# SamsungLabs/fcaf3d

Measured on AMD Instinct MI355X. Metric: scenes/sec fwd+bwd, ScanNet 100k-pt 2cm voxels, 1/2/4/8 MI355X, higher is better.
Workload: dtype f32

## Files before the change

### fcaf3d_amd/csrc/conv.hip

```cpp
#include "fc_common.h"
#include "../../include/fcaf3d_hip.h"
#ifdef FC_TRACE
__device__ unsigned long long* g_trace_buf_lds;
__device__ int g_trace_cap_lds;
extern "C" int fc_debug_trace_lds(unsigned long long* buf, int cap) {
  FC_HIP(hipMemcpyToSymbol(HIP_SYMBOL(g_trace_buf_lds), &buf, sizeof(buf)));
  FC_HIP(hipMemcpyToSymbol(HIP_SYMBOL(g_trace_cap_lds), &cap, sizeof(cap)));
  return FC_OK;
}
#define TR_BUF g_trace_buf_lds
#define TR_CAP g_trace_cap_lds
#endif
#include "fc_trace.h"

typedef float f32x16 __attribute__((ext_vector_type(16)));
typedef float f32x2 __attribute__((ext_vector_type(2)));
typedef float f32x4 __attribute__((ext_vector_type(4)));

__device__ __attribute__((aligned(16))) float g_zero_row[64];

__device__ int g_fc_prio;
extern "C" int fc_debug_set_prio(int mode) {
  FC_HIP(hipMemcpyToSymbol(HIP_SYMBOL(g_fc_prio), &mode, sizeof(mode)));
  return FC_OK;
}

static int g_bf16_fast = 0;
extern "C" int fc_set_bf16_fast(int on) {
  g_bf16_fast = on ? 1 : 0;
  return FC_OK;
}

static int g_split_mode = 2;
static inline int split_mode() { return g_bf16_fast ? 0 : g_split_mode; }
extern "C" int fc_set_split_mode(int mode) {
  if (mode != 0 && mode != 2) return FC_EINVAL;
  g_split_mode = mode;
  return FC_OK;
}
extern "C" int fc_get_split_mode(void) { return split_mode(); }
static int g_h3r = 1;
extern "C" int fc_debug_set_h3r(int mode) {
  if (mode < 0 || mode > 2) return FC_EINVAL;
  g_h3r = mode;
  return FC_OK;
}

#include <mutex>
#include "conv_tile.h"
#include "conv_f32.h"
#include "wgrad_f32.h"
#include "conv_stem.h"
#include "conv_x6.h"
#include "wgrad_x6.h"
#include "conv_h3r.h"
#include "conv_route.h"
static inline RouteEnv route_env() { return {split_mode(), g_bf16_fast, g_h3r}; }

__global__ __launch_bounds__(256) void k_amax(const f32x4* __restrict__ x, int64_t n4, const float* __restrict__ tail, int ntail,
                                              unsigned* __restrict__ slot) {
  __shared__ unsigned wm[4];
  __shared__ int last_s;
  unsigned m = 0u;
  const int64_t stride = (int64_t)gridDim.x * 256;
  for (int64_t i = (int64_t)blockIdx.x * 256 + threadIdx.x; i < n4; i += 4 * stride) {
    f32x4 v[4];
#pragma unroll
    for (int q = 0; q < 4; ++q) v[q] = i + q * stride < n4 ? x[i + q * stride] : f32x4{0.f, 0.f, 0.f, 0.f};
#pragma unroll
    for (int q = 0; q < 4; ++q)
#pragma unroll
      for (int j = 0; j < 4; ++j) { const unsigned u = __float_as_uint(v[q][j]) & 0x7fffffffu; m = (u > m && u < 0x7f800000u) ? u : m; }
  }
  if (blockIdx.x == 0 && (int)threadIdx.x < ntail) { const unsigned u = __float_as_uint(tail[threadIdx.x]) & 0x7fffffffu; m = (u > m && u < 0x7f800000u) ? u : m; }
#pragma unroll
  for (int off = 32; off > 0; off >>= 1) { const unsigned o = (unsigned)__shfl_xor((int)m, off, 64); m = o > m ? o : m; }
  if ((threadIdx.x & 63) == 0) wm[threadIdx.x >> 6] = m;
  __syncthreads();
  if (threadIdx.x == 0) {
    unsigned b = wm[0];
    for (int w = 1; w < 4; ++w) b = wm[w] > b ? wm[w] : b;
    if (b > __hip_atomic_load(&slot[1], __ATOMIC_RELAXED, __HIP_MEMORY_SCOPE_AGENT)) atomicMax(&slot[1], b);
    __threadfence();
    last_s = atomicAdd(&slot[2], 1u) == gridDim.x - 1;
    if (last_s) {
      __threadfence();
      slot[0] = atomicExch(&slot[1], 0u);
      slot[2] = 0u;
    }
  }
}

constexpr int AMAX_RING = 2048;
static unsigned* g_amax_ring[16] = {};
static unsigned g_amax_next[16] = {};
static std::mutex g_amax_ring_mu;
static int amax_ring_slot(unsigned** slot) {
  int dev = 0;
  FC_HIP(hipGetDevice(&dev));
  if (dev < 0 || dev >= 16) return FC_EINVAL;
  std::lock_guard<std::mutex> lock(g_amax_ring_mu);
  if (!g_amax_ring[dev]) {
    FC_HIP(hipMalloc((void**)&g_amax_ring[dev], (size_t)AMAX_RING * FC_AMAX_SLOT_BYTES));
    FC_HIP(hipMemset(g_amax_ring[dev], 0, (size_t)AMAX_RING * FC_AMAX_SLOT_BYTES));
  }
  const unsigned i = __atomic_fetch_add(&g_amax_next[dev], 1u, __ATOMIC_RELAXED) % AMAX_RING;
  *slot = g_amax_ring[dev] + (size_t)i * (FC_AMAX_SLOT_BYTES / 4);
  return FC_OK;
}
static int amax_launch(const float* x, int64_t n, unsigned* slot, hipStream_t stream) {
  if (n <= 0) { FC_HIP(hipMemsetAsync(slot, 0, 4, stream)); return FC_OK; }
  const int64_t n4 = n / 4;
  int64_t blocks = fc_cdiv(n4 > 0 ? n4 : 1, 256 * 8);
  if (blocks > 1024) blocks = 1024;
  k_amax<<<(unsigned)blocks, 256, 0, stream>>>(reinterpret_cast<const f32x4*>(x), n4, x + 4 * n4, (int)(n - 4 * n4), slot);
  FC_CHECK_LAUNCH();
  return FC_OK;
}
static thread_local const unsigned* t_amax_hint[2] = {nullptr, nullptr};
struct AmaxHintScope { ~AmaxHintScope() { t_amax_hint[0] = t_amax_hint[1] = nullptr; } };
static int operand_amax(const float* x, int64_t n, int which, hipStream_t stream, const unsigned** out) {
  const unsigned* h = t_amax_hint[which];
  if (h) { *out = h; return FC_OK; }
  unsigned* slot;
  int rc = amax_ring_slot(&slot);
  if (rc) return rc;
  rc = amax_launch(x, n, slot, stream);
  *out = slot;
  return rc;
}
extern "C" int fc_amax(const float* x, int64_t n, unsigned* slot, hipStream_t stream) {
  if (!slot || n < 0 || (n > 0 && !x) || ((uintptr_t)x & 15)) return FC_EINVAL;
  return amax_launch(x, n, slot, stream);
}
extern "C" int fc_conv_amax_hint(const unsigned* amax_in, const unsigned* amax_gout) {
  t_amax_hint[0] = amax_in;
  t_amax_hint[1] = amax_gout;
  return FC_OK;
}

// ... 83 lines not shown
__global__ __launch_bounds__(256) void k_sum_parts_stats(const float* __restrict__ part, float* __restrict__ out, int64_t n, int C, int S,
                                                         int RB, X6Epi epi) {
  __shared__ f32x4 sm[16 * 2 * 16];
  const int lane = threadIdx.x & 15, rl = threadIdx.x >> 4;
  const int64_t r0 = (int64_t)blockIdx.x * RB;
  const int c = blockIdx.y * 64 + lane * 4;
  const StatCh p = stat_channels(epi, c);
  f32x4 a1 = {0.f, 0.f, 0.f, 0.f}, a2 = a1;
  for (int64_t r = r0 + rl; r < r0 + RB && r < n; r += 16) {
    f32x4 a = *reinterpret_cast<const f32x4*>(part + r * C + c);
    for (int z = 1; z < S; ++z) a += *reinterpret_cast<const f32x4*>(part + ((int64_t)z * n + r) * C + c);
    *reinterpret_cast<f32x4*>(out + r * C + c) = a;
    stat_accumulate(p, epi, a, r * C + c, a1, a2);
  }
  stat_block_reduce(a1, a2, epi.stats, C, sm);
}

__global__ __launch_bounds__(256) void k_sum_pairs_stats(const float* __restrict__ part, const int* __restrict__ pos, float* __restrict__ out,
                                                         int64_t n_out, int K, int Cout, int RB, X6Epi epi) {
  __shared__ f32x4 sm[16 * 2 * 16];
  const int lane = threadIdx.x & 15, rl = threadIdx.x >> 4;
  const int64_t r0 = (int64_t)blockIdx.x * RB;
  const int c = blockIdx.y * 64 + lane * 4;
  const StatCh p = stat_channels(epi, c);
  f32x4 a1 = {0.f, 0.f, 0.f, 0.f}, a2 = a1;
  const int64_t rend = (r0 + RB < n_out) ? r0 + RB : n_out;
  for (int64_t o = r0 + rl; o < rend; o += 32) {
    const int64_t o2 = o + 16;
    const bool two = o2 < rend;
    f32x4 a = {0.f, 0.f, 0.f, 0.f}, b = a;
    for (int k0 = 0; k0 < K; k0 += 9) {
      int j[9], j2[9];
#pragma unroll
      for (int u = 0; u < 9; ++u) {
        j[u] = k0 + u < K ? pos[(int64_t)(k0 + u) * n_out + o] : -1;
        j2[u] = (two && k0 + u < K) ? pos[(int64_t)(k0 + u) * n_out + o2] : -1;
      }
      f32x4 v[9], v2[9];
#pragma unroll
      for (int u = 0; u < 9; ++u) {
        const float* src = j[u] >= 0 ? part + ((int64_t)(k0 + u) * n_out + j[u]) * Cout + c : g_zero_row + lane * 4;
        const float* src2 = j2[u] >= 0 ? part + ((int64_t)(k0 + u) * n_out + j2[u]) * Cout + c : g_zero_row + lane * 4;
        v[u] = *reinterpret_cast<const f32x4*>(src);
        v2[u] = *reinterpret_cast<const f32x4*>(src2);
      }
#pragma unroll
      for (int u = 0; u < 9; ++u) {
        if (j[u] >= 0) a += v[u];
        if (j2[u] >= 0) b += v2[u];
      }
    }
    *reinterpret_cast<f32x4*>(out + o * Cout + c) = a;
    stat_accumulate(p, epi, a, o * Cout + c, a1, a2);
    if (two) {
      *reinterpret_cast<f32x4*>(out + o2 * Cout + c) = b;
      stat_accumulate(p, epi, b, o2 * Cout + c, a1, a2);
    }
  }
  stat_block_reduce(a1, a2, epi.stats, Cout, sm);
}

static_assert(STEM_CIN == 3 && STEM_COUT == 64 && BK == 32, "conv_route.h spells these shapes out");

struct ConvArgs {
  const float *in, *W; const int *nbr, *out_index, *cnt; float* dst;
  int64_t n_rows; int K, Cin, Cout; X6Epi epi; hipStream_t stream;
};
#define FC_LAUNCH(...) __VA_ARGS__<<<grid, 256, 0, a.stream>>>(a.in, a.W, a.nbr, a.out_index, a.cnt, a.dst, a.n_rows, a.K, a.Cin, a.Cout)
#define FC_LAUNCH_EPI(...) __VA_ARGS__<<<grid, 256, 0, a.stream>>>(a.in, a.W, a.nbr, a.out_index, a.cnt, a.dst, a.n_rows, a.K, a.Cin, a.Cout, a.epi)

template <int BM, int BN, int WM>
static void launch_conv_fp32(const ConvRoute& r, const ConvArgs& a, dim3 grid) {
#define FC_LAUNCH_MFMA(KERNEL)                                                                                              \
  do { if (r.wsrc == FC_WSRC_FP32_T) FC_LAUNCH(KERNEL<BM, BN, 32, true, WM, true>); else if (a.nbr) FC_LAUNCH(KERNEL<BM, BN, 32, true, WM>); \
       else FC_LAUNCH(KERNEL<BM, BN, 32, false, WM>); } while (0)
  if (r.family == FC_FAM_MFMA) FC_LAUNCH_MFMA(k_conv_mfma);
  if constexpr (BM >= 128) {
    if (r.family == FC_FAM_MFMA_P) FC_LAUNCH_MFMA(k_conv_mfma_p);
    if (r.family == FC_FAM_GLDS) { if (a.nbr) FC_LAUNCH(k_conv_glds<BM, BN, true, WM>); else FC_LAUNCH(k_conv_glds<BM, BN, false, WM>); }
  }
#undef FC_LAUNCH_MFMA
}

template <int BM, int BN, int WM>
static void launch_conv_x6(const ConvRoute& r, const ConvArgs& a, dim3 grid) {
  if (r.family == FC_FAM_H3R) {
    if constexpr (BM == 128) {
      if (r.buf) FC_LAUNCH_EPI(k_conv_h3r<BN, true, true>);
      else if (a.nbr) FC_LAUNCH_EPI(k_conv_h3r<BN, true, false>);
      else FC_LAUNCH_EPI(k_conv_h3r<BN, false, false>);
    }
  } else if (r.wsrc == FC_WSRC_FP32_T) FC_LAUNCH_EPI(k_conv_x6<BM, BN, true, WM, 1>);
  else if (r.wsrc == FC_WSRC_FP32) { if (a.nbr) FC_LAUNCH_EPI(k_conv_x6<BM, BN, true, WM, 0>); else FC_LAUNCH_EPI(k_conv_x6<BM, BN, false, WM, 0>); }
  else if (r.mode == FC_MODE_BF16 || r.buf) {
    if constexpr (BM == 128) {
      if (r.mode == FC_MODE_BF16) { if (a.nbr) FC_LAUNCH_EPI(k_conv_x6<128, BN, true, 2, 2, 1>); else FC_LAUNCH_EPI(k_conv_x6<128, BN, false, 2, 2, 1>); }
      else if (r.mode == FC_MODE_H3) FC_LAUNCH_EPI(k_conv_x6<128, BN, true, 2, 2, 2, true>);
      else FC_LAUNCH_EPI(k_conv_x6<128, BN, true, 2, 2, 0, true>);
    }
  } else if (r.mode == FC_MODE_H3) { if (a.nbr) FC_LAUNCH_EPI(k_conv_x6<BM, BN, true, WM, 2, 2>); else FC_LAUNCH_EPI(k_conv_x6<BM, BN, false, WM, 2, 2>); }
  else { if (a.nbr) FC_LAUNCH_EPI(k_conv_x6<BM, BN, true, WM, 2>); else FC_LAUNCH_EPI(k_conv_x6<BM, BN, false, WM, 2>); }
}

static int launch_conv(const ConvRoute& r, const ConvArgs& a) {
  const dim3 grid(r.grid[0], r.grid[1], r.grid[2]);
  if (r.family == FC_FAM_STEM) {
    const size_t smem = (size_t)(STEM_ROWS * STEM_FWD_LDA + 96 * 64) * sizeof(float);
    k_stem_fwd<<<(unsigned)fc_cdiv(a.n_rows, STEM_ROWS), 256, smem, a.stream>>>(a.in, a.W, a.nbr, a.dst, nullptr, a.n_rows, a.K);
  } else if (r.family == FC_FAM_FMA) {
    k_conv_fma<<<(unsigned)fc_cdiv(a.n_rows * a.Cout, 256), 256, 0, a.stream>>>(a.in, a.W, a.nbr, a.dst, a.n_rows, a.K, a.Cin, a.Cout, r.wsrc == FC_WSRC_FP32_T ? 1 : 0);
  } else {
#define FC_TILE(BM, BN, WM) do { if (r.family >= FC_FAM_X6) launch_conv_x6<BM, BN, WM>(r, a, grid); else launch_conv_fp32<BM, BN, WM>(r, a, grid); } while (0)
    if (r.bm == 256) FC_TILE(256, 64, 4);
    else if (r.bm == 128 && r.bn == 128) FC_TILE(128, 128, 2);
    else if (r.bm == 128) FC_TILE(128, 64, 2);
    else if (r.bn == 128) launch_conv_fp32<64, 128, 2>(r, a, grid);
    else launch_conv_fp32<64, 64, 2>(r, a, grid);
#undef FC_TILE
  }
  FC_CHECK_LAUNCH();
  return FC_OK;
}
#undef FC_LAUNCH
#undef FC_LAUNCH_EPI

extern "C" {

int fc_conv_fwd_route(int64_t n_in, int64_t n_out, int K, int Cin, int Cout, int flags, int table_kind, int64_t live_tiles, int* out) {
  if (!out || n_in < 0 || n_out < 0 || K < 1 || Cin < 1 || Cout < 1) return FC_EINVAL;
  const ConvRoute r = conv_route({n_in, n_out, K, Cin, Cout}, flags, table_kind, live_tiles, route_env());
  const int f[16] = {r.family, r.bm, r.bn, r.wm, r.S, r.wsrc, r.mode, r.buf, r.epi, (int)r.grid[0], (int)r.grid[1], (int)r.grid[2]};
  for (int i = 0; i < 16; ++i) out[i] = f[i];
  return r.family == FC_FAM_INVALID ? FC_EINVAL : FC_OK;
}

int64_t fc_conv_fwd_ws_bytes(int64_t n_out, int K, int Cin, int Cout, int flags) {
  const ConvRoute r = conv_route({n_out, n_out, K, Cin, Cout}, flags, FC_TABLE_DENSE, 0, route_env());
  return r.S > 1 ? (int64_t)r.S * n_out * Cout * (int64_t)sizeof(float) : 0;
}

int64_t fc_conv_fwd_pairs_ws_bytes(int64_t n_out, int K, int Cout) {
  return (int64_t)K * n_out * Cout * (int64_t)sizeof(float);
}

int64_t fc_conv_stats_blocks(int64_t n_out, int K, int Cin, int Cout, int flags, int pairs) {
  if (n_out < 1) return 0;
  const ConvRoute r = conv_route({n_out, n_out, K, Cin, Cout}, flags, pairs ? FC_TABLE_PAIRS : FC_TABLE_DENSE, 0, route_env());
  if (r.epi == FC_EPI_NONE) return 0;
  return r.epi == FC_EPI_SUM ? fc_cdiv(n_out, fc_stat_rb(n_out)) : fc_cdiv(n_out, r.bm);
}

static int conv_impl(const float* in, const float* W, const int* nbr, const int* out_index, const int* cnt, const int* pos, float* out,
                     int64_t n_in, int64_t n_out, int K, int Cin, int Cout, int64_t live_tiles, int flags, void* ws, int64_t ws_bytes,
                     hipStream_t stream, const X6Epi* epi) {
  AmaxHintScope hint_scope;
  if (n_in < 0 || n_out < 0 || K < 1 || Cin < 1 || Cout < 1) return FC_EINVAL;
  if (n_out == 0 && !cnt) return epi ? FC_EINVAL : FC_OK;
  if (out_index && !nbr) return FC_EINVAL;
  const int table = cnt ? FC_TABLE_PAIRS : out_index ? FC_TABLE_SORTED : nbr ? FC_TABLE_DENSE : FC_TABLE_NONE;
  const ConvRoute r = conv_route({n_in, n_out, K, Cin, Cout}, flags, table | (epi ? FC_TABLE_STATS : 0), live_tiles, route_env());
  if (r.family == FC_FAM_INVALID) return FC_EINVAL;
  if (n_out == 0) return FC_OK;
  ConvArgs a = {in, W, nbr, out_index, cnt, out, n_out, K, Cin, Cout, {}, stream};
  if (r.family == FC_FAM_STEM || r.family == FC_FAM_FMA) return launch_conv(r, a);
  const bool parts = cnt || r.S > 1;
  if (parts && ws_bytes < (int64_t)r.S * n_out * Cout * (int64_t)sizeof(float)) return FC_EWS;
  if (parts) a.dst = (float*)ws;
  if (epi && r.epi == FC_EPI_KERNEL) a.epi = *epi;
  int rc = FC_OK;
  if (r.mode == FC_MODE_H3) rc = operand_amax(in, n_in * (int64_t)Cin, 0, stream, &a.epi.amax_in);
  if (rc == FC_OK) rc = launch_conv(r, a);
  if (rc != FC_OK || !parts) return rc;
  const int rb = fc_stat_rb(n_out);
  const dim3 sgrid((unsigned)fc_cdiv(n_out, rb), Cout / 64);
  if (cnt && epi) k_sum_pairs_stats<<<sgrid, 256, 0, stream>>>(a.dst, pos, out, n_out, K, Cout, rb, *epi);
  else if (cnt) k_sum_pairs<<<(unsigned)fc_cdiv(n_out * (Cout / 4), 256), 256, 0, stream>>>(a.dst, pos, out, n_out, K, Cout);
  else if (epi) k_sum_parts_stats<<<sgrid, 256, 0, stream>>>(a.dst, out, n_out, Cout, r.S, rb, *epi);
  else k_sum_parts<<<(unsigned)fc_cdiv(n_out * Cout / 4, 256), 256, 0, stream>>>(a.dst, out, n_out * Cout / 4, r.S);
  FC_CHECK_LAUNCH();
  return FC_OK;
}

static int conv_pairs_impl(const float* in, const float* W, const int* pair_in, const int* pair_cnt, const int* pair_pos, float* out,
                           int64_t n_in, int64_t n_out, int K, int Cin, int Cout, int64_t live_tiles, int flags, void* ws,
                           int64_t ws_bytes, hipStream_t stream, const X6Epi* epi) {
  if (!pair_in || !pair_cnt || !pair_pos || K > 65535) return FC_EINVAL;
  return conv_impl(in, W, pair_in, nullptr, pair_cnt, pair_pos, out, n_in, n_out, K, Cin, Cout, live_tiles, flags, ws, ws_bytes, stream, epi);
}

static X6Epi stats_epi(float* stats, const float* bn_x = nullptr, const float* mean = nullptr, const float* var = nullptr, const float* gamma = nullptr,
                       const float* beta = nullptr, float eps = 0.f, int act = 0, const float* add = nullptr, const float* bn_y = nullptr) {
  return {stats, bn_x, mean, var, gamma, beta, eps, act, add, bn_y, nullptr};
}

int fc_conv_fwd(const float* in, const float* W, const int* nbr, const int* out_index, float* out, int64_t n_in,
                int64_t n_out, int K, int Cin, int Cout, int flags, void* ws, int64_t ws_bytes, hipStream_t stream) {
// ... 311 lines not shown
```

### fcaf3d_amd/csrc/conv_h3r.h

```cpp
#pragma once

template <int BN, bool HAS_NBR, bool BUF>
__global__ __launch_bounds__(256, BN == 64 ? 4 : 3) void k_conv_h3r(
    const float* __restrict__ in, const float* __restrict__ W, const int* __restrict__ nbr,
    const int* __restrict__ out_index, const int* __restrict__ cnt, float* __restrict__ out, int64_t n_out, int K, int Cin,
    int Cout, X6Epi epi) {
  constexpr int BM = 128;
  constexpr int TN = BN / 32;
  constexpr int NG = BN / 64;
  constexpr int GU = 2 * 64 * 4;
  constexpr int BU = 3 * BN / 64;
  __shared__ u32x4 Bs[2][NG * GU];
  __shared__ unsigned int kmask_s;
  float* __restrict__ stats = epi.stats;

  const int tid = threadIdx.x, lane = tid & 63;
  const int wave = __builtin_amdgcn_readfirstlane(tid >> 6);
  const int r = lane & 31, h = lane >> 5;
  int64_t bx = blockIdx.x;
  const int n0 = blockIdx.y * BN;
  int S = gridDim.z, z = blockIdx.z;
  int kbase = 0;
  if (cnt) {
    const PairTile pt = tile_pair_walk<BM>(cnt, K, bx, z);
    bx = pt.bx; z = pt.z;
    const int64_t stride = n_out;
    n_out = cnt[z];
    if (bx * BM >= n_out) return;
    nbr += (int64_t)z * stride;
    kbase = z;
    out += (int64_t)z * stride * Cout;
    K = 1; S = 1; z = 0;
  }
  const int64_t m0 = bx * BM;
  const float h3_sa = h3_scale(fc_amax_read(epi.amax_in));
  const float h3_inv = h3_unscale(h3_sa, h3_scale(fc_amax_read(reinterpret_cast<const unsigned*>(W) + X6_IMG_AMAX_WORD)));

  f32x16 acc[TN];
#pragma unroll
  for (int j = 0; j < TN; ++j)
#pragma unroll
    for (int e = 0; e < 16; ++e) acc[j][e] = 0.f;

  const unsigned int kmask = (unsigned int)__builtin_amdgcn_readfirstlane((int)tile_offset_mask<BM, HAS_NBR>(&kmask_s, nbr, m0, n_out, z, K, S, tid, lane));
  constexpr unsigned X6_DEAD = 0x80000000u;

  if (kmask) {
    const int nst = __popc(kmask) * (Cin / 32);
    unsigned int rem = kmask;
    int lk = __ffs(rem) - 1;
    rem &= rem - 1;
    int lnk = rem ? __ffs(rem) - 1 : lk;
    if (rem) rem &= rem - 1;
    int lc0 = 0;
    bool sw = false;
    f32x4 av[4];
    u32x4 bi[BU];
    int vcur, vnxt;
    const int rows_here = (int)((n_out - m0) < BM ? (n_out - m0) : BM);
    const int lrow = wave * 32 + r;
    const __amdgpu_buffer_rsrc_t rn = __builtin_amdgcn_make_buffer_rsrc(const_cast<int*>(nbr), 0, 0x7fffffff, 0x00020000);
    const unsigned irow = (lrow < rows_here ? (unsigned)(m0 + lrow) : 0u) * 4u;
    auto fetch_idx = [&](int kk) -> int {
      if (BUF && HAS_NBR) return (int)__builtin_amdgcn_raw_buffer_load_b32(rn, (int)irow, (int)((unsigned)kk * (unsigned)n_out * 4u), 0);
      const int64_t row = lrow < rows_here ? m0 + lrow : 0;
      return HAS_NBR ? nbr[(int64_t)kk * n_out + row] : (int)row;
    };
    vcur = fetch_idx(lk);
    vnxt = fetch_idx(lnk);
    unsigned ocur = 0u;
    auto row_offset = [&]() {
      ocur = (vcur >= 0 && lrow < rows_here) ? (unsigned)vcur * (unsigned)(Cin * 4) + (unsigned)(h * 32) : X6_DEAD;
    };
    if (BUF) row_offset();
    const __amdgpu_buffer_rsrc_t ra = __builtin_amdgcn_make_buffer_rsrc(const_cast<float*>(in), 0, (int)X6_DEAD, 0x00020000);
    const __amdgpu_buffer_rsrc_t rb = __builtin_amdgcn_make_buffer_rsrc(const_cast<float*>(W), 0, -1, 0x00020000);
    const u32x4* img = reinterpret_cast<const u32x4*>(W);
    const int nslab = Cin / 32, ngrp = Cout / 64;
    auto load_stage = [&]() {
      if (sw) {
        sw = false;
        lk = lnk;
        vcur = vnxt;
        if (rem) {
          lnk = __ffs(rem) - 1;
          rem &= rem - 1;
        }
        vnxt = fetch_idx(lnk);
        if (BUF) row_offset();
      }
      if (BUF) {
        const unsigned boff = (((unsigned)(kbase + lk) * (unsigned)nslab + (unsigned)(lc0 / 32)) * (unsigned)ngrp + (unsigned)(n0 / 64)) * (unsigned)(X6_GROUP_U16 * 16);
#pragma unroll
        for (int i = 0; i < BU; ++i)
          if (i % 3 != 2) bi[i] = __builtin_amdgcn_raw_buffer_load_b128(rb, tid * 16, (int)(boff + 4096u * i), 0);
#pragma unroll
        for (int q = 0; q < 4; ++q)
          av[q] = __builtin_bit_cast(f32x4, __builtin_amdgcn_raw_buffer_load_b128(ra, (int)(ocur + (unsigned)(64 * (q >> 1) + 16 * (q & 1))), lc0 * 4, 0));
        return;
      }
      const u32x4* src = img + (((int64_t)(kbase + lk) * nslab + lc0 / 32) * ngrp + n0 / 64) * X6_GROUP_U16 + tid;
#pragma unroll
      for (int i = 0; i < BU; ++i)
        if (i % 3 != 2) bi[i] = src[256 * i];
      const bool live = vcur >= 0 && lrow < rows_here;
      const float* rowp = live ? in + (int64_t)vcur * Cin + lc0 + 8 * h : g_zero_row;
#pragma unroll
      for (int q = 0; q < 4; ++q) av[q] = *reinterpret_cast<const f32x4*>(rowp + (live ? 16 * (q >> 1) + 4 * (q & 1) : 4 * q));
    };
    u32x4 fa[2][2];
    auto split_rows = [&]() {
#pragma unroll
      for (int b = 0; b < 2; ++b) {
        unsigned p0[4], p1[4];
#pragma unroll
        for (int q = 0; q < 2; ++q) {
          h3_split2s(av[2 * b + q][0], av[2 * b + q][1], h3_sa, p0[2 * q], p1[2 * q]);
          h3_split2s(av[2 * b + q][2], av[2 * b + q][3], h3_sa, p0[2 * q + 1], p1[2 * q + 1]);
        }
        fa[b][0] = u32x4{p0[0], p0[1], p0[2], p0[3]};
        fa[b][1] = u32x4{p1[0], p1[1], p1[2], p1[3]};
      }
    };
    auto store_weights = [&](int buf) {
#pragma unroll
      for (int i = 0; i < BU; ++i)
        if (i % 3 != 2) Bs[buf][(i / 3) * GU + (i % 3) * 256 + tid] = bi[i];
    };
    load_stage();
    store_weights(0);
    split_rows();
    const int swz = (r >> 2) & 3;
    int b_slot[2];
#pragma unroll
    for (int b = 0; b < 2; ++b) b_slot[b] = r * 4 + ((2 * b + h) ^ swz);
    for (int st = 0; st < nst; ++st) {
      const int cur = st & 1;
      __syncthreads();
      if (st + 1 < nst) {
        lc0 += 32;
        if (lc0 >= Cin) {
          lc0 = 0;
          sw = true;
        }
      }
      load_stage();
      __builtin_amdgcn_sched_barrier(0);
#pragma unroll
      for (int b = 0; b < 2; ++b) {
#pragma unroll
        for (int pb = 1; pb >= 0; --pb) {
          u32x4 fb[TN];
#pragma unroll
          for (int j = 0; j < TN; ++j) fb[j] = Bs[cur][(j >> 1) * GU + pb * 256 + (j & 1) * 32 * 4 + b_slot[b]];
#pragma unroll
          for (int pa = 1 - pb; pa >= 0; --pa)
#pragma unroll
            for (int j = 0; j < TN; ++j) acc[j] = H3_MFMA(fa[b][pa], fb[j], acc[j]);
        }
      }
      store_weights(cur ^ 1);
      split_rows();
    }
  }
#pragma unroll
  for (int j = 0; j < TN; ++j)
#pragma unroll
    for (int e = 0; e < 16; ++e) acc[j][e] *= h3_inv;

  float* dst = out + (int64_t)z * n_out * Cout + n0 + 2 * r;
  int orow[16];
#pragma unroll
  for (int e = 0; e < 16; ++e) {
    const int64_t row = m0 + wave * 32 + (e & 3) + 8 * (e >> 2) + 4 * h;
    int o = -1;
    if (row < n_out) o = out_index ? out_index[row] : (int)row;
    orow[e] = o;
  }
  if (stats) {
    const bool bwd = epi.bn_x != nullptr;
    const bool from_y = bwd && epi.bn_y != nullptr && epi.act != 0;
    float mu[TN], is[TN], ga[TN], be[TN];
#pragma unroll
    for (int j = 0; j < TN; ++j) {
      const int col = n0 + (j >> 1) * 64 + 2 * r + (j & 1);
      mu[j] = 0.f; is[j] = 1.f; ga[j] = 1.f; be[j] = 0.f;
      if (bwd) {
        mu[j] = epi.mean[col];
        is[j] = 1.f / sqrtf(epi.var[col] + epi.eps);
        ga[j] = epi.gamma ? epi.gamma[col] : 1.f;
        be[j] = epi.beta ? epi.beta[col] : 0.f;
      }
    }
    float s1[TN], s2[TN];
#pragma unroll
    for (int j = 0; j < TN; ++j) { s1[j] = 0.f; s2[j] = 0.f; }
#pragma unroll
    for (int e0 = 0; e0 < 16; e0 += 4) {
      float xv[4][TN], av2[4][TN], yv[4][TN];
#pragma unroll
      for (int u = 0; u < 4; ++u) {
        const int o = orow[e0 + u];
#pragma unroll
        for (int j = 0; j < TN; ++j) { xv[u][j] = 0.f; av2[u][j] = 0.f; yv[u][j] = 0.f; }
        if (bwd && o >= 0) {
#pragma unroll
          for (int g = 0; g < NG; ++g) {
            const int64_t at = (int64_t)o * Cout + n0 + g * 64 + 2 * r;
            const f32x2 t = *reinterpret_cast<const f32x2*>(epi.bn_x + at);
            xv[u][2 * g] = t[0]; xv[u][2 * g + 1] = t[1];
            if (epi.add) { const f32x2 a2 = *reinterpret_cast<const f32x2*>(epi.add + at); av2[u][2 * g] = a2[0]; av2[u][2 * g + 1] = a2[1]; }
            if (from_y) { const f32x2 y2 = *reinterpret_cast<const f32x2*>(epi.bn_y + at); yv[u][2 * g] = y2[0]; yv[u][2 * g + 1] = y2[1]; }
          }
        }
      }
#pragma unroll
      for (int u = 0; u < 4; ++u) {
        if (bwd && orow[e0 + u] < 0) continue;
#pragma unroll
        for (int j = 0; j < TN; ++j) {
          float t1, t2;
          x6_epi_terms(bwd, bwd ? av2[u][j] + acc[j][e0 + u] : acc[j][e0 + u], xv[u][j], mu[j], is[j], ga[j], be[j], epi.act, from_y,
                       yv[u][j], t1, t2);
          s1[j] += t1;
          s2[j] += t2;
        }
      }
    }
#pragma unroll
    for (int j = 0; j < TN; ++j) {
      s1[j] += __shfl_xor(s1[j], 32, 64);
      s2[j] += __shfl_xor(s2[j], 32, 64);
    }
    __syncthreads();
    float* red = reinterpret_cast<float*>(&Bs[0][0]);
    if (h == 0) {
#pragma unroll
      for (int j = 0; j < TN; ++j) {
        const int cl = (j >> 1) * 64 + 2 * r + (j & 1);
        red[(wave * BN + cl) * 2 + 0] = s1[j];
        red[(wave * BN + cl) * 2 + 1] = s2[j];
      }
    }
    __syncthreads();
    if (tid < BN) {
      float a = 0.f, b = 0.f;
#pragma unroll
      for (int w = 0; w < 4; ++w) { a += red[(w * BN + tid) * 2 + 0]; b += red[(w * BN + tid) * 2 + 1]; }
      stats[((int64_t)blockIdx.x * 2 + 0) * Cout + n0 + tid] = a;
      stats[((int64_t)blockIdx.x * 2 + 1) * Cout + n0 + tid] = b;
    }
  }
#pragma unroll
  for (int e = 0; e < 16; ++e) {
    if (orow[e] >= 0) {
#pragma unroll
      for (int g = 0; g < NG; ++g) {
        f32x2 v = {acc[2 * g][e], acc[2 * g + 1][e]};
        *reinterpret_cast<f32x2*>(dst + (int64_t)orow[e] * Cout + g * 64) = v;
      }
    }
  }
}
```

### fcaf3d_amd/csrc/conv_route.h

```cpp
#ifndef FC_CONV_ROUTE_H
#define FC_CONV_ROUTE_H
#include "fc_common.h"
#include "../../include/fcaf3d_hip.h"

struct RouteEnv { int split_mode, bf16_fast, h3r; };
struct ConvShape { int64_t n_in, n_out; int K, Cin, Cout; };

struct ConvRoute {
  int family;
  int bm, bn, wm;
  int S;
  int wsrc, mode, buf, epi;
  unsigned grid[3];
};
struct WgradRoute {
  int family;
  int bm, bn, ko, bkr;
  int table, mode, S;
  int64_t rps;
  int wbuf;
  unsigned grid_y;
};

static inline int flag_bm(int flags) { return (flags >> FC_CONV_BM_SHIFT) & FC_CONV_TILE_MASK; }
static inline int flag_bn(int flags) { return (flags >> FC_CONV_BN_SHIFT) & FC_CONV_TILE_MASK; }
static inline int flag_s(int flags) { return (flags >> FC_CONV_S_SHIFT) & FC_CONV_S_MASK; }
static inline bool below_2gb(uint64_t bytes) { return bytes < (1ull << 31) - 4096u; }

static inline bool stem_shape(int K, int Cin, int Cout, int flags) { return !(flags & FC_CONV_FMA) && Cin == 3 && Cout == 64 && K <= 27; }

static inline int offset_split(int64_t tiles, int K) {
  if (K <= 1 || tiles >= 384) return 1;
  return (int)(1024 / tiles < K ? 1024 / tiles : K);
}

static inline ConvRoute conv_route(const ConvShape& s, int flags, int table, int64_t live_tiles, const RouteEnv& env) {
  const bool stats = (table & FC_TABLE_STATS) != 0;
  table &= ~FC_TABLE_STATS;
  const bool pairs = table == FC_TABLE_PAIRS, gather = table != FC_TABLE_NONE, split = (flags & FC_CONV_SPLIT) != 0;
  const bool image = split && (flags & FC_CONV_IMAGE);
  const bool wt = (flags & FC_CONV_WT) && !image;
  const int64_t n = s.n_out > 0 ? s.n_out : 1;
  const int K = s.K, Cin = s.Cin, Cout = s.Cout;
  ConvRoute r = {};
  r.family = FC_FAM_INVALID;
  r.wsrc = image ? FC_WSRC_IMAGE : wt ? FC_WSRC_FP32_T : FC_WSRC_FP32;
  if (!gather && (K != 1 || s.n_in != s.n_out)) return r;
  if ((flags & FC_CONV_WT) && !gather) return r;
  const bool mfma = Cin % 32 == 0 && Cout % 64 == 0 && (pairs || (!(flags & FC_CONV_FMA) && K <= 32));
  if (pairs && !mfma) return r;
  if (stats && !(mfma && split)) return r;
  r.bn = (Cout % 128 == 0) ? 128 : 64;
  if (pairs) {
    if (flag_bn(flags) == 1) r.bn = 64;
    r.bm = 128;
    r.S = K;
  } else {
    r.bm = (n > 64 && fc_cdiv(n, 128) * (Cout / r.bn) >= 4) ? 128 : 64;
    if (Cout == 64 && fc_cdiv(n, 256) >= 1024 && !split) r.bm = 256;
    const int fbm = flag_bm(flags), fbn = flag_bn(flags);
    if (fbm) r.bm = fbm == 1 ? 64 : (fbm == 2 ? 128 : 256);
    if (fbn && (Cout % (fbn == 1 ? 64 : 128) == 0)) r.bn = fbn == 1 ? 64 : 128;
    if (r.bm == 256) r.bn = 64;
    if (split && mfma && r.bm == 64) r.bm = 128;
    r.S = mfma ? offset_split(fc_cdiv(n, r.bm) * (Cout / r.bn), K) : 1;
    if (flag_s(flags)) r.S = flag_s(flags) > K ? K : flag_s(flags);
  }
  r.wm = r.bm == 256 ? 4 : 2;
  if (stem_shape(K, Cin, Cout, flags) && !(flags & FC_CONV_WT) && table == FC_TABLE_DENSE) { r.family = FC_FAM_STEM; return r; }
  if (!mfma && table != FC_TABLE_SORTED && !(flags & FC_CONV_IMAGE)) r.family = FC_FAM_FMA;
  if (!mfma) return r;
  r.grid[0] = (unsigned)fc_cdiv(n, r.bm), r.grid[1] = (unsigned)(Cout / r.bn), r.grid[2] = (unsigned)r.S;
  if (pairs && live_tiles > 0) r.grid[0] = (unsigned)live_tiles, r.grid[2] = 1;
  if (split) {
    r.family = FC_FAM_X6;
    r.mode = !image ? FC_MODE_SIX : (env.bf16_fast && r.bm == 128) ? FC_MODE_BF16 : env.split_mode == 2 ? FC_MODE_H3 : FC_MODE_SIX;
    if (r.mode == FC_MODE_H3 && r.bm == 128 && (env.h3r == 2 || (env.h3r == 1 && r.bn == 128))) r.family = FC_FAM_H3R;
    r.buf = image && gather && r.bm == 128 && r.mode != FC_MODE_BF16 && !(flags & FC_CONV_FLAT) &&
            below_2gb((uint64_t)s.n_in * (uint64_t)Cin * 4u) && below_2gb((uint64_t)K * (uint64_t)s.n_out * 4u);
    r.epi = (pairs || r.S > 1) ? FC_EPI_SUM : FC_EPI_KERNEL;
    return r;
  }
  const int64_t wgs = (int64_t)r.grid[0] * r.grid[1] * r.grid[2];
  r.mode = FC_MODE_FP32;
  if (flags & FC_CONV_GLDS) r.family = FC_FAM_GLDS;
  else if (flags & FC_CONV_PIPE_ON) r.family = FC_FAM_MFMA_P;
  else if ((flags & FC_CONV_PIPE_OFF) || (pairs && live_tiles <= 0)) r.family = FC_FAM_MFMA;
  else if (wgs >= 1536 || wgs <= 768) r.family = FC_FAM_MFMA_P;
  else r.family = (r.grid[2] > 1 && !(flags & FC_CONV_GLDS_OFF)) ? FC_FAM_GLDS : FC_FAM_MFMA;
  if (r.family == FC_FAM_GLDS && wt) r.family = FC_FAM_MFMA;
  if (r.bm == 64) r.family = FC_FAM_MFMA;
  return r;
}

#define WGRAD_KO 3

static inline WgradRoute wgrad_route(const ConvShape& s, int flags, int table, const RouteEnv& env) {
  const int64_t n = s.n_out > 0 ? s.n_out : 1;
  const int K = s.K, Cin = s.Cin, Cout = s.Cout, fbm = flag_bm(flags), fbn = flag_bn(flags);
  const bool dense = table == FC_TABLE_DENSE, pairs = table == FC_TABLE_PAIRS, split = (flags & FC_CONV_SPLIT) != 0;
  if (pairs) flags &= ~FC_CONV_WGRAD_DEEP;
  WgradRoute r = {};
  r.family = FC_WFAM_INVALID;
  r.table = table, r.ko = 1, r.bkr = 32, r.mode = FC_MODE_FP32;
  if (table == FC_TABLE_SORTED || (table == FC_TABLE_NONE && (K != 1 || s.n_in != s.n_out))) return r;
  const bool mfma = !(flags & FC_CONV_FMA) && Cin % 64 == 0 && Cout % 64 == 0;
  if (pairs && !mfma) return r;
  if (stem_shape(K, Cin, Cout, flags)) {
    r.family = dense ? FC_WFAM_STEM : FC_WFAM_FMA;
    r.rps = 1024, r.S = (int)fc_cdiv(n, 1024), r.grid_y = dense ? 1 : (unsigned)K;
    return r;
  }
  const bool multi = dense && mfma && !(flags & FC_CONV_WGRAD_MULTI_OFF) && K % WGRAD_KO == 0 && n >= 4096 &&
                     (!(flags & FC_CONV_WGRAD_MULTI_FIRST) || (Cin == 64 && n >= 32768));
  const bool x6t = mfma && split && (multi || !dense);
  const int wide = (Cout % 128 == 0) ? 128 : 64;
  r.bm = 64;
  r.bn = wide;
  if (fbm == 2 && Cin % 128 == 0) r.bm = 128;
  if (fbn == 1) r.bn = 64;
  if (fbn == 2 && Cout % 128 == 0) r.bn = 128;
  if (split && !dense && Cin % 128 == 0) r.bm = 128;
  int64_t sp = 1728 / (mfma ? (int64_t)K * (Cin / r.bm) * (Cout / r.bn) : (int64_t)K);
  if (multi) {
    constexpr int round_wide = 256, round_narrow = 512;
    sp = (wide == 128 ? round_wide : round_narrow) / ((int64_t)(K / WGRAD_KO) * (Cin / 64) * (Cout / wide));
  }
  const int64_t max_by_rows = fc_cdiv(n, mfma ? 512 : 2048);
  sp = sp > max_by_rows ? max_by_rows : sp;
  sp = sp > 256 ? 256 : sp < 1 ? 1 : sp;
  if (flag_s(flags)) sp = flag_s(flags);
  r.rps = fc_align(fc_cdiv(n, sp), 64);
  r.S = (int)fc_cdiv(n, r.rps);
  if (!mfma) { r.family = FC_WFAM_FMA, r.grid_y = (unsigned)K; return r; }
  if (x6t) {
    r.family = FC_WFAM_X6T;
    r.mode = env.bf16_fast ? FC_MODE_BF16 : env.split_mode == 2 ? FC_MODE_H3 : FC_MODE_SIX;
    r.bn = wide;
    if (multi) r.bm = 64, r.ko = WGRAD_KO;
    else if (r.bm == 128 && r.bn == 128 && (int64_t)r.S * K * (Cin / 128) * (Cout / 128) < 512) r.bm = 64;
    r.wbuf = !(flags & FC_CONV_FLAT) && below_2gb((uint64_t)s.n_in * (uint64_t)Cin * 4u) && below_2gb((uint64_t)s.n_out * (uint64_t)Cout * 4u) &&
             s.n_in < (1 << 24) && s.n_out < (1 << 24) && below_2gb((uint64_t)K * (uint64_t)s.n_out * 4u);
  } else if (multi) {
    r.family = FC_WFAM_MULTI, r.bm = 64, r.bn = wide, r.ko = WGRAD_KO;
  } else {
    if (pairs) r.bm = 64;
    const bool wpipe = r.bm == 64 && !(flags & FC_CONV_WGRAD_DEEP) && !(flags & FC_CONV_WGRAD_PIPE_OFF) &&
                       ((flags & FC_CONV_WGRAD_PIPE_ON) || (pairs && r.bn == 128));
    r.family = wpipe ? FC_WFAM_MFMA_P : FC_WFAM_MFMA;
    if (!wpipe && dense && (flags & FC_CONV_WGRAD_DEEP) && r.bm == 64) r.bkr = 64;
  }
  r.grid_y = (unsigned)((K / r.ko) * (Cin / r.bm) * (Cout / r.bn));
  return r;
}
#endif
```

### include/fcaf3d_hip.h

```cpp
#ifndef FCAF3D_HIP_H
#define FCAF3D_HIP_H
#include <stdint.h>

#ifndef __HIP_PLATFORM_AMD__
typedef struct ihipStream_t* hipStream_t;
#endif

#ifdef __cplusplus
extern "C" {
#endif

#define FC_ABI_VERSION 19
#ifndef FC_AMAX_SLOT_BYTES
#define FC_AMAX_SLOT_BYTES 2048
#endif
int fc_abi_version(void);


int fc_voxelize(const float* points, int64_t n, int pt_stride, int batch_idx, float voxel_size, float feat_div,
                int nfeat, int* coords, float* feats, hipStream_t stream);

int fc_augment_voxelize(const float* points, int64_t n_src, int pt_stride, const int* sample_idx, int64_t n_out,
                        const float* xform_host, int batch_idx, float voxel_size, float feat_div, int nfeat, int* coords,
                        float* feats, float* points_out, hipStream_t stream);
// ... 263 lines not shown
                      int kind, float* loss, float* iou, float* dpred, hipStream_t stream);

int fc_head_split_fwd(const float* y, int ld, const float* bias, const float* scale_dev, int64_t n, int n_reg, int n_cls,
                      float* centerness, float* bbox_pred, float* cls_score, float* cls_max, hipStream_t stream);
int fc_head_split_bwd(const float* y, int ld, const float* scale_dev, const float* bbox_pred, const float* g_centerness,
                      const float* g_bbox, const float* g_cls, int64_t n, int n_reg, int n_cls, float* gy,
                      float* gscale_row, hipStream_t stream);
int64_t fc_head_split_bwd_sums_ws_bytes(int64_t n);
int fc_head_split_bwd_sums(const float* y, int ld, const float* scale_dev, const float* bbox_pred, const float* g_centerness,
                           const float* g_bbox, const float* g_cls, int64_t n, int n_reg, int n_cls, float* gy, float* gbias,
                           float* gscale, void* ws, int64_t ws_bytes, hipStream_t stream);

int fc_sort_v(const float* vertices, const unsigned char* mask, const int* num_valid, int64_t n_pairs, int* idx,
              hipStream_t stream);

int64_t fc_assign_ws_bytes(int B, int M, int L);
int fc_assign_targets(const float* points, const int* scene, const int* level, int64_t N, const float* boxes,
                      const long long* labels, const int* box_count, int B, int M, int L, const int* order,
                      const int* seg_start, int limit, int topk, float* centerness_t, float* bbox_t, long long* labels_out,
                      void* ws, int64_t ws_bytes, hipStream_t stream);


int64_t fc_nms_bev_ws_bytes(int nseg, int stride);
int fc_nms_bev(const float* boxes, const int* counts_dev, int nseg, int stride, float thresh, int rotated,
               unsigned long long* mask_ws, int64_t ws_bytes, int* keep, int* keep_count, hipStream_t stream);
int fc_boxes_iou_bev(const float* boxes_a, int n, const float* boxes_b, int m, int rotated, float* out,
                     hipStream_t stream);


#define FC_MERGE_TO_BOTTOM 1
#define FC_MERGE_WITH_YAW 2
#define FC_MERGE_XF_FLIP_H (1ull << 32)
#define FC_MERGE_XF_FLIP_V (1ull << 33)
int64_t fc_merge_sorted_segments_ws_bytes(int nseg_out, int max_total);
int fc_merge_sorted_segments(const int64_t* desc, int nseg_out, int K, const int* counts_dev, const int* keep, int keep_stride,
                             const int64_t* ord, int ord_stride, const float* scores, int score_stride, const float* boxes,
                             int flags, int max_total, int cap, float* out_boxes, float* out_scores, int* out_src,
                             int* out_count, int stride_out, void* ws, int64_t ws_bytes, hipStream_t stream);


#define FC_VOTE_ROTATED 1
#define FC_VOTE_WITH_YAW 2
int fc_vote_boxes(const float* boxes, const float* scores, const int* counts_dev, int nseg, int stride, int max_count,
                  const int* keep, const int* keep_counts_dev, int keep_stride, int max_keep, float vote_thr, int flags,
                  float* out_boxes, int* out_members, hipStream_t stream);


#define FC_EVAL_DET_BOTTOM 1
int64_t fc_eval_match_ws_bytes(int64_t n_det, int64_t n_gt, int n_thr);
int fc_eval_match(const float* det_boxes, int det_dim , const float* det_scores, const int64_t* det_labels,
                  const float* gt_boxes , const int* gt_labels,
                  const int64_t* seg , int n_scenes,
                  int64_t n_det, int64_t n_gt, const double* thr , int n_thr, int flags,
                  float* best_iou, int* best_gt, unsigned char* tp_bits, void* ws, int64_t ws_bytes, hipStream_t stream);


int64_t fc_grad_norm_ws_bytes(int64_t n);
int fc_grad_norm(const float* g, int64_t n, float max_norm, float* out, void* ws, int64_t ws_bytes, hipStream_t stream);
int fc_adamw_step(float* p, const float* g, float* m, float* v, int64_t n, float lr, float beta1, float beta2, float eps,
                  float weight_decay, float bias_correction1, float bias_correction2, const float* norm_and_clip,
                  hipStream_t stream);

#define FC_ADAMW_MAX_RUNS 1024
int64_t fc_adamw_groups_table_bytes(int R);
int fc_adamw_groups_pack(const int64_t* begin, const float* lr_mult, const float* decay_mult, int R, int64_t n, void* out,
                         int64_t out_bytes);
int fc_adamw_step_groups(float* p, const float* g, float* m, float* v, int64_t n, float lr, float beta1, float beta2, float eps,
                         float weight_decay, float bias_correction1, float bias_correction2, const float* norm_and_clip,
                         const void* table_dev, int R, hipStream_t stream);

int fc_adamw_ema_step(float* p, const float* g, float* m, float* v, float* ema, int64_t n, float lr, float beta1, float beta2,
                      float eps, float weight_decay, float bias_correction1, float bias_correction2, const float* norm_and_clip,
                      const void* table_dev, int R, float ema_mu, float ema_keep, hipStream_t stream);
int fc_swap_f32(float* a, float* b, int64_t n, hipStream_t stream);

int fc_set_bf16_fast(int on);

int fc_set_split_mode(int mode);
int fc_get_split_mode(void);
int fc_amax(const float* x, int64_t n, unsigned* slot, hipStream_t stream);
int fc_conv_amax_hint(const unsigned* amax_in, const unsigned* amax_gout);
int fc_amax_out_hint(unsigned* amax_word);
int fc_debug_set_h3r(int mode);


int fc_exec_op_words(void);
int64_t fc_exec_probe_read(float* ms, int64_t* meta, int64_t cap);
int fc_exec_map_words(void);
int fc_exec(const int64_t* ops, int64_t op_begin, int64_t op_end, const int64_t* addr, const int64_t* dims, const int64_t* maps,
            const int64_t* streams, const int64_t* ws, const int64_t* ws_bytes, int64_t* ws_need, const int64_t* cfg);

#ifdef __cplusplus
}
#endif
#endif
```

Measured before the change: 538.5.

## Add 128x256 wide-N tile variant of h3r conv kernel for large wide shapes

Adds a BN=256 instantiation of the h3r split-precision conv kernel and routes wide, pair-driven convolutions with Cin>=256 and enough tiles to it, halving the grid along Cout. Wider N tiles reuse each gathered A fragment across twice as many MFMA columns, reducing gather/LDS traffic per FLOP. To limit register pressure the B-fragment loads and the BN-stats epilogue are processed in sub-groups, and occupancy is lowered to 2 waves per SIMD. It risks spills and lower occupancy hiding latency, and is controlled by a new debug knob.

```diff
diff --git a/fcaf3d_amd/csrc/conv.hip b/fcaf3d_amd/csrc/conv.hip
--- a/fcaf3d_amd/csrc/conv.hip
+++ b/fcaf3d_amd/csrc/conv.hip
@@ -43,6 +43,13 @@
 extern "C" int fc_debug_set_h3r(int mode) {
   if (mode < 0 || mode > 2) return FC_EINVAL;
   g_h3r = mode;
+  return FC_OK;
+}
+
+static int g_h3r_wide = 1;
+extern "C" int fc_debug_set_h3r_wide(int mode) {
+  if (mode < 0 || mode > 2) return FC_EINVAL;
+  g_h3r_wide = mode;
   return FC_OK;
 }
 
@@ -55,7 +62,7 @@
 #include "wgrad_x6.h"
 #include "conv_h3r.h"
 #include "conv_route.h"
-static inline RouteEnv route_env() { return {split_mode(), g_bf16_fast, g_h3r}; }
+static inline RouteEnv route_env() { return {split_mode(), g_bf16_fast, g_h3r, g_h3r_wide}; }
 
 __global__ __launch_bounds__(256) void k_amax(const f32x4* __restrict__ x, int64_t n4, const float* __restrict__ tail, int ntail,
                                               unsigned* __restrict__ slot) {
@@ -305,14 +312,17 @@
 #undef FC_LAUNCH_MFMA
 }
 
+template <int BN>
+static void launch_conv_h3r(const ConvRoute& r, const ConvArgs& a, dim3 grid) {
+  if (r.buf) FC_LAUNCH_EPI(k_conv_h3r<BN, true, true>);
+  else if (a.nbr) FC_LAUNCH_EPI(k_conv_h3r<BN, true, false>);
+  else FC_LAUNCH_EPI(k_conv_h3r<BN, false, false>);
+}
+
 template <int BM, int BN, int WM>
 static void launch_conv_x6(const ConvRoute& r, const ConvArgs& a, dim3 grid) {
   if (r.family == FC_FAM_H3R) {
-    if constexpr (BM == 128) {
-      if (r.buf) FC_LAUNCH_EPI(k_conv_h3r<BN, true, true>);
-      else if (a.nbr) FC_LAUNCH_EPI(k_conv_h3r<BN, true, false>);
-      else FC_LAUNCH_EPI(k_conv_h3r<BN, false, false>);
-    }
+    if constexpr (BM == 128) launch_conv_h3r<BN>(r, a, grid);
   } else if (r.wsrc == FC_WSRC_FP32_T) FC_LAUNCH_EPI(k_conv_x6<BM, BN, true, WM, 1>);
   else if (r.wsrc == FC_WSRC_FP32) { if (a.nbr) FC_LAUNCH_EPI(k_conv_x6<BM, BN, true, WM, 0>); else FC_LAUNCH_EPI(k_conv_x6<BM, BN, false, WM, 0>); }
   else if (r.mode == FC_MODE_BF16 || r.buf) {
@@ -335,6 +345,7 @@
   } else {
 #define FC_TILE(BM, BN, WM) do { if (r.family >= FC_FAM_X6) launch_conv_x6<BM, BN, WM>(r, a, grid); else launch_conv_fp32<BM, BN, WM>(r, a, grid); } while (0)
     if (r.bm == 256) FC_TILE(256, 64, 4);
+    else if (r.bn == 256) launch_conv_h3r<256>(r, a, grid);
     else if (r.bm == 128 && r.bn == 128) FC_TILE(128, 128, 2);
     else if (r.bm == 128) FC_TILE(128, 64, 2);
     else if (r.bn == 128) launch_conv_fp32<64, 128, 2>(r, a, grid);
diff --git a/fcaf3d_amd/csrc/conv_h3r.h b/fcaf3d_amd/csrc/conv_h3r.h
--- a/fcaf3d_amd/csrc/conv_h3r.h
+++ b/fcaf3d_amd/csrc/conv_h3r.h
@@ -1,13 +1,15 @@
 #pragma once
 
 template <int BN, bool HAS_NBR, bool BUF>
-__global__ __launch_bounds__(256, BN == 64 ? 4 : 3) void k_conv_h3r(
+__global__ __launch_bounds__(256, BN == 64 ? 4 : BN == 256 ? 2 : 3) void k_conv_h3r(
     const float* __restrict__ in, const float* __restrict__ W, const int* __restrict__ nbr,
     const int* __restrict__ out_index, const int* __restrict__ cnt, float* __restrict__ out, int64_t n_out, int K, int Cin,
     int Cout, X6Epi epi) {
   constexpr int BM = 128;
   constexpr int TN = BN / 32;
   constexpr int NG = BN / 64;
+  constexpr int FG = 4;
+  constexpr int SJ = 2;
   constexpr int GU = 2 * 64 * 4;
   constexpr int BU = 3 * BN / 64;
   __shared__ u32x4 Bs[2][NG * GU];
@@ -150,13 +152,26 @@
       for (int b = 0; b < 2; ++b) {
 #pragma unroll
         for (int pb = 1; pb >= 0; --pb) {
-          u32x4 fb[TN];
-#pragma unroll
-          for (int j = 0; j < TN; ++j) fb[j] = Bs[cur][(j >> 1) * GU + pb * 256 + (j & 1) * 32 * 4 + b_slot[b]];
-#pragma unroll
-          for (int pa = 1 - pb; pa >= 0; --pa)
-#pragma unroll
-            for (int j = 0; j < TN; ++j) acc[j] = H3_MFMA(fa[b][pa], fb[j], acc[j]);
+          if constexpr (TN <= 4) {
+            u32x4 fb[TN];
+#pragma unroll
+            for (int j = 0; j < TN; ++j) fb[j] = Bs[cur][(j >> 1) * GU + pb * 256 + (j & 1) * 32 * 4 + b_slot[b]];
+#pragma unroll
+            for (int pa = 1 - pb; pa >= 0; --pa)
+#pragma unroll
+              for (int j = 0; j < TN; ++j) acc[j] = H3_MFMA(fa[b][pa], fb[j], acc[j]);
+          } else {
+#pragma unroll
+            for (int j0 = 0; j0 < TN; j0 += FG) {
+              u32x4 fb[FG];
+#pragma unroll
+              for (int j = j0; j < j0 + FG; ++j) fb[j - j0] = Bs[cur][(j >> 1) * GU + pb * 256 + (j & 1) * 32 * 4 + b_slot[b]];
+#pragma unroll
+              for (int pa = 1 - pb; pa >= 0; --pa)
+#pragma unroll
+                for (int j = j0; j < j0 + FG; ++j) acc[j] = H3_MFMA(fa[b][pa], fb[j - j0], acc[j]);
+            }
+          }
         }
       }
       store_weights(cur ^ 1);
@@ -180,50 +195,103 @@
   if (stats) {
     const bool bwd = epi.bn_x != nullptr;
     const bool from_y = bwd && epi.bn_y != nullptr && epi.act != 0;
-    float mu[TN], is[TN], ga[TN], be[TN];
-#pragma unroll
-    for (int j = 0; j < TN; ++j) {
-      const int col = n0 + (j >> 1) * 64 + 2 * r + (j & 1);
-      mu[j] = 0.f; is[j] = 1.f; ga[j] = 1.f; be[j] = 0.f;
-      if (bwd) {
-        mu[j] = epi.mean[col];
-        is[j] = 1.f / sqrtf(epi.var[col] + epi.eps);
-        ga[j] = epi.gamma ? epi.gamma[col] : 1.f;
-        be[j] = epi.beta ? epi.beta[col] : 0.f;
-      }
-    }
     float s1[TN], s2[TN];
-#pragma unroll
-    for (int j = 0; j < TN; ++j) { s1[j] = 0.f; s2[j] = 0.f; }
-#pragma unroll
-    for (int e0 = 0; e0 < 16; e0 += 4) {
-      float xv[4][TN], av2[4][TN], yv[4][TN];
-#pragma unroll
-      for (int u = 0; u < 4; ++u) {
-        const int o = orow[e0 + u];
-#pragma unroll
-        for (int j = 0; j < TN; ++j) { xv[u][j] = 0.f; av2[u][j] = 0.f; yv[u][j] = 0.f; }
-        if (bwd && o >= 0) {
-#pragma unroll
-          for (int g = 0; g < NG; ++g) {
-            const int64_t at = (int64_t)o * Cout + n0 + g * 64 + 2 * r;
-            const f32x2 t = *reinterpret_cast<const f32x2*>(epi.bn_x + at);
-            xv[u][2 * g] = t[0]; xv[u][2 * g + 1] = t[1];
-            if (epi.add) { const f32x2 a2 = *reinterpret_cast<const f32x2*>(epi.add + at); av2[u][2 * g] = a2[0]; av2[u][2 * g + 1] = a2[1]; }
-            if (from_y) { const f32x2 y2 = *reinterpret_cast<const f32x2*>(epi.bn_y + at); yv[u][2 * g] = y2[0]; yv[u][2 * g + 1] = y2[1]; }
-          }
-        }
-      }
-#pragma unroll
-      for (int u = 0; u < 4; ++u) {
-        if (bwd && orow[e0 + u] < 0) continue;
-#pragma unroll
-        for (int j = 0; j < TN; ++j) {
-          float t1, t2;
-          x6_epi_terms(bwd, bwd ? av2[u][j] + acc[j][e0 + u] : acc[j][e0 + u], xv[u][j], mu[j], is[j], ga[j], be[j], epi.act, from_y,
-                       yv[u][j], t1, t2);
-          s1[j] += t1;
-          s2[j] += t2;
+    if constexpr (TN <= 4) {
+      float mu[TN], is[TN], ga[TN], be[TN];
+#pragma unroll
+      for (int j = 0; j < TN; ++j) {
+        const int col = n0 + (j >> 1) * 64 + 2 * r + (j & 1);
+        mu[j] = 0.f; is[j] = 1.f; ga[j] = 1.f; be[j] = 0.f;
+        if (bwd) {
+          mu[j] = epi.mean[col];
+          is[j] = 1.f / sqrtf(epi.var[col] + epi.eps);
+          ga[j] = epi.gamma ? epi.gamma[col] : 1.f;
+          be[j] = epi.beta ? epi.beta[col] : 0.f;
+        }
+      }
+#pragma unroll
+      for (int j = 0; j < TN; ++j) { s1[j] = 0.f; s2[j] = 0.f; }
+#pragma unroll
+      for (int e0 = 0; e0 < 16; e0 += 4) {
+        float xv[4][TN], av2[4][TN], yv[4][TN];
+#pragma unroll
+        for (int u = 0; u < 4; ++u) {
+          const int o = orow[e0 + u];
+#pragma unroll
+          for (int j = 0; j < TN; ++j) { xv[u][j] = 0.f; av2[u][j] = 0.f; yv[u][j] = 0.f; }
+          if (bwd && o >= 0) {
+#pragma unroll
+            for (int g = 0; g < NG; ++g) {
+              const int64_t at = (int64_t)o * Cout + n0 + g * 64 + 2 * r;
+              const f32x2 t = *reinterpret_cast<const f32x2*>(epi.bn_x + at);
+              xv[u][2 * g] = t[0]; xv[u][2 * g + 1] = t[1];
+              if (epi.add) { const f32x2 a2 = *reinterpret_cast<const f32x2*>(epi.add + at); av2[u][2 * g] = a2[0]; av2[u][2 * g + 1] = a2[1]; }
+              if (from_y) { const f32x2 y2 = *reinterpret_cast<const f32x2*>(epi.bn_y + at); yv[u][2 * g] = y2[0]; yv[u][2 * g + 1] = y2[1]; }
+            }
+          }
+        }
+#pragma unroll
+        for (int u = 0; u < 4; ++u) {
+          if (bwd && orow[e0 + u] < 0) continue;
+#pragma unroll
+          for (int j = 0; j < TN; ++j) {
+            float t1, t2;
+            x6_epi_terms(bwd, bwd ? av2[u][j] + acc[j][e0 + u] : acc[j][e0 + u], xv[u][j], mu[j], is[j], ga[j], be[j], epi.act, from_y,
+                         yv[u][j], t1, t2);
+            s1[j] += t1;
+            s2[j] += t2;
+          }
+        }
+      }
+    } else {
+#pragma unroll
+      for (int j0 = 0; j0 < TN; j0 += SJ) {
+        float mu[SJ], is[SJ], ga[SJ], be[SJ];
+#pragma unroll
+        for (int j = j0; j < j0 + SJ; ++j) {
+          const int col = n0 + (j >> 1) * 64 + 2 * r + (j & 1), i = j - j0;
+          mu[i] = 0.f; is[i] = 1.f; ga[i] = 1.f; be[i] = 0.f;
+          if (bwd) {
+            mu[i] = epi.mean[col];
+            is[i] = 1.f / sqrtf(epi.var[col] + epi.eps);
+            ga[i] = epi.gamma ? epi.gamma[col] : 1.f;
+            be[i] = epi.beta ? epi.beta[col] : 0.f;
+          }
+        }
+#pragma unroll
+        for (int j = j0; j < j0 + SJ; ++j) { s1[j] = 0.f; s2[j] = 0.f; }
+#pragma unroll
+        for (int e0 = 0; e0 < 16; e0 += 4) {
+          float xv[4][SJ], av2[4][SJ], yv[4][SJ];
+#pragma unroll
+          for (int u = 0; u < 4; ++u) {
+            const int o = orow[e0 + u];
+#pragma unroll
+            for (int i = 0; i < SJ; ++i) { xv[u][i] = 0.f; av2[u][i] = 0.f; yv[u][i] = 0.f; }
+            if (bwd && o >= 0) {
+#pragma unroll
+              for (int g = 0; g < SJ / 2; ++g) {
+                const int64_t at = (int64_t)o * Cout + n0 + (j0 / 2 + g) * 64 + 2 * r;
+                const f32x2 t = *reinterpret_cast<const f32x2*>(epi.bn_x + at);
+                xv[u][2 * g] = t[0]; xv[u][2 * g + 1] = t[1];
+                if (epi.add) { const f32x2 a2 = *reinterpret_cast<const f32x2*>(epi.add + at); av2[u][2 * g] = a2[0]; av2[u][2 * g + 1] = a2[1]; }
+                if (from_y) { const f32x2 y2 = *reinterpret_cast<const f32x2*>(epi.bn_y + at); yv[u][2 * g] = y2[0]; yv[u][2 * g + 1] = y2[1]; }
+              }
+            }
+          }
+#pragma unroll
+          for (int u = 0; u < 4; ++u) {
+            if (bwd && orow[e0 + u] < 0) continue;
+#pragma unroll
+            for (int j = j0; j < j0 + SJ; ++j) {
+              const int i = j - j0;
+              float t1, t2;
+              x6_epi_terms(bwd, bwd ? av2[u][i] + acc[j][e0 + u] : acc[j][e0 + u], xv[u][i], mu[i], is[i], ga[i], be[i], epi.act, from_y,
+                           yv[u][i], t1, t2);
+              s1[j] += t1;
+              s2[j] += t2;
+            }
+          }
         }
       }
     }
diff --git a/fcaf3d_amd/csrc/conv_route.h b/fcaf3d_amd/csrc/conv_route.h
--- a/fcaf3d_amd/csrc/conv_route.h
+++ b/fcaf3d_amd/csrc/conv_route.h
@@ -3,7 +3,7 @@
 #include "fc_common.h"
 #include "../../include/fcaf3d_hip.h"
 
-struct RouteEnv { int split_mode, bf16_fast, h3r; };
+struct RouteEnv { int split_mode, bf16_fast, h3r, h3r_wide; };
 struct ConvShape { int64_t n_in, n_out; int K, Cin, Cout; };
 
 struct ConvRoute {
@@ -32,6 +32,11 @@
 static inline int offset_split(int64_t tiles, int K) {
   if (K <= 1 || tiles >= 384) return 1;
   return (int)(1024 / tiles < K ? 1024 / tiles : K);
+}
+
+static inline bool h3r_wide_shape(const ConvShape& s, bool pairs) {
+  const int64_t rows = s.n_in < s.n_out ? s.n_in : s.n_out;
+  return pairs && s.Cin >= 256 && fc_cdiv(rows > 0 ? rows : 1, 128) * s.K * (s.Cout / 256) >= 512;
 }
 
 static inline ConvRoute conv_route(const ConvShape& s, int flags, int table, int64_t live_tiles, const RouteEnv& env) {
@@ -76,6 +81,9 @@
     r.family = FC_FAM_X6;
     r.mode = !image ? FC_MODE_SIX : (env.bf16_fast && r.bm == 128) ? FC_MODE_BF16 : env.split_mode == 2 ? FC_MODE_H3 : FC_MODE_SIX;
     if (r.mode == FC_MODE_H3 && r.bm == 128 && (env.h3r == 2 || (env.h3r == 1 && r.bn == 128))) r.family = FC_FAM_H3R;
+    if (r.family == FC_FAM_H3R && r.bn == 128 && Cout % 256 == 0 && !flag_bn(flags) &&
+        (env.h3r_wide == 2 || (env.h3r_wide == 1 && h3r_wide_shape(s, pairs))))
+      r.bn = 256, r.grid[1] = (unsigned)(Cout / 256);
     r.buf = image && gather && r.bm == 128 && r.mode != FC_MODE_BF16 && !(flags & FC_CONV_FLAT) &&
             below_2gb((uint64_t)s.n_in * (uint64_t)Cin * 4u) && below_2gb((uint64_t)K * (uint64_t)s.n_out * 4u);
     r.epi = (pairs || r.S > 1) ? FC_EPI_SUM : FC_EPI_KERNEL;
diff --git a/include/fcaf3d_hip.h b/include/fcaf3d_hip.h
--- a/include/fcaf3d_hip.h
+++ b/include/fcaf3d_hip.h
@@ -369,6 +369,7 @@
 int fc_conv_amax_hint(const unsigned* amax_in, const unsigned* amax_gout);
 int fc_amax_out_hint(unsigned* amax_word);
 int fc_debug_set_h3r(int mode);
+int fc_debug_set_h3r_wide(int mode);
 
 
 int fc_exec_op_words(void);
```

Measured after the change: 541.5 (median of 6 runs). No clear change (+0.5%).
